# stardist/stardist

Hardware: AMD Instinct MI355X
Metric: predict_instances() Mpix/s (2D) + Mvox/s (3D) end-to-end at 1/2/4/8 GPU (higher is better)
Workload: dtype f32

## Files before the change

### stardist_amd/csrc/conv3x3_f16.hip

```cpp
#include <stdlib.h>

#include "common.h"
#include "conv3x3_device.h"
#include "stardist_hip.h"

#ifdef SD_CONV_PROFILE
__device__ unsigned long long g_conv_prof[20];
#define PROF_DECL unsigned long long pf_t = __builtin_amdgcn_s_memtime(), pf_acc[16] = {}; const unsigned long long pf_t0 = pf_t; unsigned long long pf_units = 0
#define PROF(k) do { const unsigned long long n_ = __builtin_amdgcn_s_memtime(); pf_acc[k] += n_ - pf_t; pf_t = n_; } while (0)
#define PROF_UNIT() (++pf_units)
#define PROF_END() do { if (threadIdx.x == 0) { atomicAdd(&g_conv_prof[0], __builtin_amdgcn_s_memtime() - pf_t0); \
  for (int k_ = 0; k_ < 16; ++k_) atomicAdd(&g_conv_prof[1 + k_], pf_acc[k_]); atomicAdd(&g_conv_prof[19], pf_units); } } while (0)
#else
#define PROF_DECL
#define PROF(k)
#define PROF_UNIT()
#define PROF_END()
#endif

#ifndef SD_CONV_EXP
#define SD_CONV_EXP 3
#endif

namespace {
// ... 90 lines not shown
  r.rsrc = __builtin_amdgcn_make_buffer_rsrc((void*)((k ? S1.p : S0.p) + (unsigned long long)(fl * 4)), 0, (int)HALO_RANGE, 0x00020000);
  r.ty0 = T.ty0; r.tx0 = T.tx0; r.H = zin ? d.H : 0; r.W = d.W;
  r.k = k; r.in = (int)(T.interior && zin);
  return r;
}

constexpr int WREG = (HWSUB_BYTES / 16 + THREADS - 1) / THREADS;
static_assert(WREG * THREADS == HWSUB_BYTES / 16, "a sub-unit's weights are a whole number of 16-byte elements per thread");
__device__ __forceinline__ void weights_fetch(const Params& P, int g, int u, int dy, v4f (&wreg)[WREG], int tid) {
  const char* blk = (const char*)P.wp + (((size_t)g * P.n_units + u) * 3 + dy) * HWSUB_BYTES;
  const __amdgpu_buffer_rsrc_t r = __builtin_amdgcn_make_buffer_rsrc((void*)uniform64((unsigned long long)blk), 0, HWSUB_BYTES, 0x00020000);
#pragma unroll
  for (int n = 0; n < WREG; ++n) wreg[n] = __builtin_bit_cast(v4f, __builtin_amdgcn_raw_buffer_load_b128(r, tid * 16, n * THREADS * 16, 0));
}
__device__ __forceinline__ void weights_store(char* __restrict__ wnext, const v4f (&wreg)[WREG], int tid) {
#pragma unroll
  for (int n = 0; n < WREG; ++n) ((v4f*)wnext)[tid + n * THREADS] = wreg[n];
}

__device__ __forceinline__ void split2_pair(float a, float b, unsigned& hi, unsigned& lo, float& amax) {
  const f32x2 x = {a, b};
  const f16x2 h = __builtin_convertvector(x, f16x2);
  hi = __builtin_bit_cast(unsigned, h);
  const f32x2 r = (x - __builtin_convertvector(h, f32x2)) * 2048.f;
  lo = __builtin_bit_cast(unsigned, __builtin_convertvector(r, f16x2));
  amax = __builtin_fmaxf(amax, __builtin_fmaxf(__builtin_fabsf(a), __builtin_fabsf(b)));
}
__device__ __forceinline__ void split_elem(const v4f x, u32x2 (&pl)[2], float& amax) {
  unsigned a[2], b[2];
  split2_pair(x.x, x.y, a[0], a[1], amax);
  split2_pair(x.z, x.w, b[0], b[1], amax);
#pragma unroll
  for (int p = 0; p < 2; ++p) {
    asm volatile("" : "+v"(a[p]), "+v"(b[p]));
    pl[p].x = a[p]; pl[p].y = b[p];
  }
}
__device__ __forceinline__ void store_planes(const StageH& st, char* __restrict__ tileH, const u32x2 (&pk)[PRE_F4][2], int tid) {
#pragma unroll
  for (int n = 0; n < PRE_F4; ++n)
    if (n < PRE_F4 - 1 || tid < TILE_F4 - (PRE_F4 - 1) * THREADS) {
#pragma unroll
      for (int p = 0; p < 2; ++p) *(u32x2*)(tileH + lds_off_of(st.tyx[n], tid) + p * 64) = pk[n][p];
    }
}

__device__ __forceinline__ void store_copy(const StageH& st, char* __restrict__ tileH, const v4f (&pre)[PRE_F4], int tid) {
#pragma unroll
  for (int n = 0; n < PRE_F4; ++n)
    if (n < PRE_F4 - 1 || tid < TILE_F4 - (PRE_F4 - 1) * THREADS) {
      const int pb = n < (TILE_F4 >> 8) ? 32 * n + ((tid >> 3) & 7) * 4 + ((tid >> 6) & 3) : (tid >> 3) + n * (THREADS / 8);
      *(v4f*)(tileH + pb * HPIX + (tid & 7) * 16) = pre[n];
    }
}

template <int NV, int NLD, class Extra>
__device__ __forceinline__ void compute_sub(const char* __restrict__ tileH, const char* __restrict__ w, int dy, f32x16 (&acc0)[2], f32x16 (&acc1)[2],
                                            int wave, int i, int h, Extra extra) {
  u32x4 A[2][2][2], B[2][2];
  const char* arow = tileH + (wave * 2 + dy) * HALO_W * HPIX;
#define SD_LOAD_GROUP_H(gi, buf)                                                                                        \
  do {                                                                                                                   \
    const int dx_ = (gi) >> 1, b_ = (gi) & 1;                                                                            \
    if (!(SD_CONV_EXP & 4) || (gi) < 2) {                                                                               \
    _Pragma("unroll") for (int p = 0; p < 2; ++p)                                                                        \
      _Pragma("unroll") for (int pl = 0; pl < 2; ++pl) A[buf][p][pl] = *(const u32x4*)(arow + htile_off(p, i + dx_, pl, b_, h)); \
    }                                                                                                                    \
    if (!(SD_CONV_EXP & 8) || (gi) < 2) {                                                                               \
    _Pragma("unroll") for (int pl = 0; pl < 2; ++pl) B[buf][pl] = *(const u32x4*)(w + hw_off(dx_, b_, pl, h, i));        \
    }                                                                                                                    \
  } while (0)
  SD_LOAD_GROUP_H(0, 0);
#pragma unroll
  for (int gi = 0; gi < 6; ++gi) {
    const int buf = gi & 1;
    if (gi + 1 < 6) SD_LOAD_GROUP_H(gi + 1, buf ^ 1);
    __builtin_amdgcn_sched_barrier(0);
    extra(gi);
    const f16x8 bh = __builtin_bit_cast(f16x8, B[buf][0]), bl = __builtin_bit_cast(f16x8, B[buf][1]);
    {
      const f16x8 a0h = __builtin_bit_cast(f16x8, A[buf][0][0]), a0l = __builtin_bit_cast(f16x8, A[buf][0][1]);
      const f16x8 a1h = __builtin_bit_cast(f16x8, A[buf][1][0]), a1l = __builtin_bit_cast(f16x8, A[buf][1][1]);
#if SD_CONV_EXP & 2
      acc1[0] = __builtin_amdgcn_mfma_f32_32x32x16_f16(a0h, bl, acc1[0], 0, 0, 0);
      acc1[1] = __builtin_amdgcn_mfma_f32_32x32x16_f16(a1h, bl, acc1[1], 0, 0, 0);
      acc0[0] = __builtin_amdgcn_mfma_f32_32x32x16_f16(a0h, bh, acc0[0], 0, 0, 0);
      acc1[0] = __builtin_amdgcn_mfma_f32_32x32x16_f16(a0l, bh, acc1[0], 0, 0, 0);
      acc1[1] = __builtin_amdgcn_mfma_f32_32x32x16_f16(a1l, bh, acc1[1], 0, 0, 0);
      acc0[1] = __builtin_amdgcn_mfma_f32_32x32x16_f16(a1h, bh, acc0[1], 0, 0, 0);
#else
      acc1[0] = __builtin_amdgcn_mfma_f32_32x32x16_f16(a0h, bl, acc1[0], 0, 0, 0);
      acc1[0] = __builtin_amdgcn_mfma_f32_32x32x16_f16(a0l, bh, acc1[0], 0, 0, 0);
      acc0[0] = __builtin_amdgcn_mfma_f32_32x32x16_f16(a0h, bh, acc0[0], 0, 0, 0);
      acc1[1] = __builtin_amdgcn_mfma_f32_32x32x16_f16(a1h, bl, acc1[1], 0, 0, 0);
      acc1[1] = __builtin_amdgcn_mfma_f32_32x32x16_f16(a1l, bh, acc1[1], 0, 0, 0);
      acc0[1] = __builtin_amdgcn_mfma_f32_32x32x16_f16(a1h, bh, acc0[1], 0, 0, 0);
#endif
    }
    if (NV > 0 || NLD > 0) {
#pragma unroll
      for (int k = 0; k < 6; ++k) {
        __builtin_amdgcn_sched_group_barrier(0x008, 1, 0);
        if (NV > 0) __builtin_amdgcn_sched_group_barrier(0x002, NV, 0);
        if (NLD > 0 && k % (6 / NLD) == 0) __builtin_amdgcn_sched_group_barrier(0x020, 1, 0);
      }
    }
    __builtin_amdgcn_sched_barrier(0);
  }
#undef SD_LOAD_GROUP_H
}

template <bool RES, bool DOT, bool NOST = false>
__device__ __forceinline__ void store_tile(const Params& P, const f32x16 (&acc0)[2], const f32x16 (&acc1)[2], float* __restrict__ scr, int g, int tz,
                                           int ty, int tx, int wave, int lane) {
  const int i = lane & 31, h = lane >> 5;
  const int px = lane >> 3, c4 = lane & 7;
  const unsigned pix_bytes = (unsigned)P.c_out * 4u, res_bytes = (unsigned)P.res_stride * 4u;
  const unsigned chan_off = (unsigned)(g * 32 + c4 * 4) * 4u;
#pragma unroll
  for (int p = 0; p < 2; ++p) {
    const int y = ty + wave * 2 + p;
    if (y >= P.H) continue;
    const size_t row = ((size_t)tz * P.H + y) * P.W;
    const __amdgpu_buffer_rsrc_t ro =
        __builtin_amdgcn_make_buffer_rsrc((void*)uniform64((unsigned long long)(P.out + row * P.c_out)), 0, (int)((unsigned)P.W * pix_bytes), 0x00020000);
    __amdgpu_buffer_rsrc_t rr = ro;
    if (RES && P.res)
      rr = __builtin_amdgcn_make_buffer_rsrc((void*)uniform64((unsigned long long)(P.res + row * P.res_stride)), 0, (int)((unsigned)P.W * res_bytes), 0x00020000);
    __amdgpu_buffer_rsrc_t rd = ro;
    if (DOT)
      rd = __builtin_amdgcn_make_buffer_rsrc((void*)uniform64((unsigned long long)(P.dotp + row * (size_t)(P.c_out >> 2))), 0, (int)((unsigned)P.W * (unsigned)P.c_out), 0x00020000);
#pragma unroll
    for (int q = 0; q < 2; ++q) {
#pragma unroll
      for (int r8 = 0; r8 < 8; ++r8) {
        const int r = q * 8 + r8;
        const int pl = (r8 & 3) + 8 * (r8 >> 2) + 4 * h;
        scr[pl * 32 + i] = acc0[p][r] + acc1[p][r] * 4.8828125e-4f;
      }
#pragma unroll
      for (int n = 0; n < 2; ++n) {
        v4f v = *(const v4f*)(scr + n * 256 + lane * 4);
        const unsigned x = (unsigned)(tx + q * 16 + n * 8 + px);
        if (RES && P.res) v += __builtin_bit_cast(v4f, __builtin_amdgcn_raw_buffer_load_b128(rr, (int)(x * res_bytes + chan_off), 0, 0));
        if (P.act == 1) { v.x = fmaxf(v.x, 0.f); v.y = fmaxf(v.y, 0.f); v.z = fmaxf(v.z, 0.f); v.w = fmaxf(v.w, 0.f); }
        const int so = (int)(x * pix_bytes + chan_off);
        if (!NOST) __builtin_amdgcn_raw_buffer_store_b128(__builtin_bit_cast(u32x4, v), ro, so, 0, 0);
        if (DOT) {
          const v4f hw = *(const v4f*)(scr + (4 - wave) * 512 + c4 * 4);
          float d = v.x * hw.x;
          d += v.y * hw.y; d += v.z * hw.z; d += v.w * hw.w;
          __builtin_amdgcn_raw_buffer_store_b32(__builtin_bit_cast(unsigned, d), rd, so >> 2, 0, 0);
        }
      }
    }
  }
}

__device__ __forceinline__ void store_tile_split(const Params& P, const f32x16 (&acc0)[2], const f32x16 (&acc1)[2], float* __restrict__ scr, int g, int tz,
                                                 int ty, int tx, int wave, int lane, float& amax) {
  const int i = lane & 31, h = lane >> 5;
  const int pr = lane >> 2, o = lane & 3;
  const unsigned pix_bytes = (unsigned)P.c_out * 4u;
  const unsigned chan_off = (unsigned)(g * 128 + o * 16);
  const int wofs = ((i >> 2) & 1) * 256 + (i >> 3) * 4 + (i & 3);
#pragma unroll
  for (int p = 0; p < 2; ++p) {
    const int y = ty + wave * 2 + p;
    if (y >= P.H) continue;
    const size_t row = ((size_t)tz * P.H + y) * P.W;
    const __amdgpu_buffer_rsrc_t ro =
        __builtin_amdgcn_make_buffer_rsrc((void*)uniform64((unsigned long long)(P.out + row * P.c_out)), 0, (int)((unsigned)P.W * pix_bytes), 0x00020000);
#pragma unroll
    for (int q = 0; q < 2; ++q) {
#pragma unroll
      for (int r8 = 0; r8 < 8; ++r8) {
        const int r = q * 8 + r8;
        const int pl = (r8 & 3) + 8 * (r8 >> 2) + 4 * h;
        scr[pl * 16 + wofs] = acc0[p][r] + acc1[p][r] * 4.8828125e-4f;
      }
      v4f va = *(const v4f*)(scr + lane * 4), vb = *(const v4f*)(scr + 256 + lane * 4);
      if (P.act == 1) {
        va.x = fmaxf(va.x, 0.f); va.y = fmaxf(va.y, 0.f); va.z = fmaxf(va.z, 0.f); va.w = fmaxf(va.w, 0.f);
        vb.x = fmaxf(vb.x, 0.f); vb.y = fmaxf(vb.y, 0.f); vb.z = fmaxf(vb.z, 0.f); vb.w = fmaxf(vb.w, 0.f);
      }
      unsigned hw[4], lw[4];
      split2_pair(va.x, va.y, hw[0], lw[0], amax);
      split2_pair(va.z, va.w, hw[1], lw[1], amax);
      split2_pair(vb.x, vb.y, hw[2], lw[2], amax);
      split2_pair(vb.z, vb.w, hw[3], lw[3], amax);
      const u32x4 hi = {hw[0], hw[1], hw[2], hw[3]}, lo = {lw[0], lw[1], lw[2], lw[3]};
      const int so = (int)((unsigned)(tx + q * 16 + pr) * pix_bytes + chan_off);
      __builtin_amdgcn_raw_buffer_store_b128(hi, ro, so, 0, 0);
      __builtin_amdgcn_raw_buffer_store_b128(lo, ro, so + 64, 0, 0);
    }
  }
}

template <bool RES, int WPE, bool DOT = false, bool INP = false, bool OUTP = false, bool NOST = false>
__global__ void __launch_bounds__(THREADS) __attribute__((amdgpu_waves_per_eu(WPE, WPE))) k_conv3_f16(const Params P) {
  static_assert(!(OUTP && (RES || DOT)), "a split16 output has neither residual nor fused head");
  static_assert(!NOST || DOT, "only the fused-head form can do without its tile store");
  extern __shared__ float4 smem4h[];
  char* W = (char*)smem4h;
  char* tileH = W + 2 * HWSUB_BYTES;
  const int tid = threadIdx.x, lane = tid & 63;
  const int wave = __builtin_amdgcn_readfirstlane(tid >> 6);
  float* scr = (float*)(tileH + HTILE_BYTES) + wave * 512;
  int g, q, Q;
  wg_slot(P, g, q, Q);
  if (q >= P.n_tiles) return;
  if (DOT && tid < 32) ((float*)(tileH + HTILE_BYTES) + 4 * 512)[tid] = P.dotw[g * 32 + tid];
  const float bias_r = P.bias ? P.bias[g * 32 + (lane & 31)] : 0.f;
  StageH st;
  stage_init_h(st, tid);
  const unsigned q4off = (unsigned)(tid & 7) * 16u;
  constexpr bool PREOFF = INP && (SD_CONV_EXP & 1);
  unsigned offk[PREOFF ? 2 : 1][PREOFF ? PRE_F4 : 1];
  if constexpr (PREOFF) {
#pragma unroll
    for (int k = 0; k < 2; ++k) {
      const Src S = P.kind[k];
      const unsigned rowb = (unsigned)((P.W >> S.shx) * S.stride * 4), pixb = (unsigned)(S.stride * 4);
#pragma unroll
      for (int n = 0; n < PRE_F4; ++n) {
        const int ty = (int)(st.tyx[n] & 255u), tx = (int)(st.tyx[n] >> 8);
        offk[k][n] = (unsigned)(((ty - S.shy) >> S.shy) + S.shy) * rowb + ((unsigned)(((tx - S.shx) >> S.shx) + S.shx) * pixb + q4off);
      }
    }
  }
  const SrcS S0 = src_scalars(P, 0), S1 = src_scalars(P, 1);
  DimS dim;
  dim.D = __builtin_amdgcn_readfirstlane(P.D); dim.H = __builtin_amdgcn_readfirstlane(P.H); dim.W = __builtin_amdgcn_readfirstlane(P.W);
  dim.kz = __builtin_amdgcn_readfirstlane(P.kz); dim.n0 = __builtin_amdgcn_readfirstlane(P.n_chunks0);
  TileAddr Tc, Tn;
  TileWalk walk;
  walk_init(P, q, Q, walk);
  tile_at(P, walk, Tc);
  Tn = Tc;
  float amax = 0.f, amax_out = 0.f;
  {
    v4f pre[PRE_F4], wreg[WREG];
    weights_fetch(P, g, 0, 0, wreg, tid);
    {
      const HaloRsrc hs = halo_rsrc(P, halo_base(P, Tc, 0), Tc);
#pragma unroll
      for (int n = 0; n < PRE_F4; ++n) pre[n] = halo_load_one(hs, halo_off_one(hs, st.tyx[n], q4off));
    }
    weights_store(W, wreg, tid);
    if (INP) store_copy(st, tileH, pre, tid);
    else {
      u32x2 pk[PRE_F4][2];
#pragma unroll
      for (int n = 0; n < PRE_F4; ++n) split_elem(pre[n], pk[n], amax);
      store_planes(st, tileH, pk, tid);
    }
  }
  __syncthreads();
  PROF_DECL;
  int wb = 0;
  for (int t = q; t < P.n_tiles; t += Q) {
    f32x16 acc0[2], acc1[2];
#pragma unroll
    for (int p = 0; p < 2; ++p)
#pragma unroll
      for (int r = 0; r < 16; ++r) { acc0[p][r] = bias_r; acc1[p][r] = 0.f; }
    for (int u = 0; u < P.n_units; ++u) {
      const bool last = u == P.n_units - 1;
      const int tn = last ? t + Q : t, un = last ? 0 : u + 1;
      const bool have = tn < P.n_tiles;
      v4f pre[PRE_F4];
      unsigned addr[PRE_F4];
      u32x2 pk[INP ? 1 : PRE_F4][2];
      HaloRsrc hs;
      UnitS us;
#pragma unroll
      for (int dy = 0; dy < 3; ++dy) {
        const bool lastdy = dy == 2, have_w = lastdy ? have : true;
        v4f wreg[WREG];
        weights_fetch(P, g, lastdy ? (have ? un : u) : u, lastdy ? (have ? 0 : dy) : dy + 1, wreg, tid);
        __builtin_amdgcn_sched_barrier(0);
        PROF(dy);
        if (!PREOFF && dy == 0 && last && have) { walk_step(P, walk); tile_at(P, walk, Tn); }
        __builtin_amdgcn_sched_barrier(0);
        if (dy == 0) PROF(14);
        const char* wcur = W + wb * HWSUB_BYTES;
        if (PREOFF && dy == 1 && !us.in) {
#pragma unroll
          for (int n = 0; n < PRE_F4; ++n) {
            const int ty = (int)(st.tyx[n] & 255u), tx = (int)(st.tyx[n] >> 8);
            const bool inside = (int)((unsigned)(us.ty0 + ty) < (unsigned)us.H) & (int)((unsigned)(us.tx0 + tx) < (unsigned)us.W);
            addr[n] = inside ? addr[n] : HALO_OUTSIDE;
          }
        }
        if (dy == 0 && PREOFF) {
          compute_sub<1, 0>(tileH, wcur, dy, acc0, acc1, wave, lane & 31, lane >> 5, [&](int gi) {
            if (gi == 0) {
              if (last && have) { walk_step(P, walk); tile_at_s(S0, S1, dim, walk, Tn); }
              us = unit_scalars(S0, S1, dim, tile_select(last && have, Tc, Tn), have ? un : u);
            } else {
              const bool k1 = us.k != 0;
#pragma unroll
              for (int n = (gi - 1) * 3; n < (gi - 1) * 3 + 3; ++n)
                if (n < PRE_F4) { unsigned a = k1 ? offk[1][PREOFF ? n : 0] : offk[0][PREOFF ? n : 0]; asm volatile("" : "+v"(a)); addr[n] = a; }
            }
          });
        } else if (dy == 0) {
          const TileAddr T = tile_select(last && have, Tc, Tn);
          const HaloBase hb = halo_base(P, T, have ? un : u);
          hs = halo_rsrc(P, hb, T);
          PROF(8);
          compute_sub<5, 0>(tileH, wcur, dy, acc0, acc1, wave, lane & 31, lane >> 5, [&](int gi) {
#pragma unroll
            for (int n = gi * 2; n < gi * 2 + 2; ++n)
              if (n < PRE_F4) addr[n] = halo_off_one(hs, st.tyx[n], q4off);
          });
        } else if (dy == 1) {
          compute_sub<0, 2>(tileH, wcur, dy, acc0, acc1, wave, lane & 31, lane >> 5, [&](int gi) {
#pragma unroll
            for (int n = gi * 2; n < gi * 2 + 2; ++n)
              if (n < PRE_F4) pre[n] = PREOFF ? __builtin_bit_cast(v4f, __builtin_amdgcn_raw_buffer_load_b128(us.rsrc, (int)addr[n], 0, 0)) : halo_load_one(hs, addr[n]);
          });
        } else if (INP) {
          compute_sub<0, 0>(tileH, wcur, dy, acc0, acc1, wave, lane & 31, lane >> 5, [&](int) {});
        } else {
          compute_sub<6, 0>(tileH, wcur, dy, acc0, acc1, wave, lane & 31, lane >> 5, [&](int gi) {
#pragma unroll
            for (int n = (gi - 2) * 3; n < (gi - 2) * 3 + 3; ++n)
              if (gi >= 2 && n < PRE_F4) split_elem(pre[n], pk[INP ? 0 : n], amax);
          });
        }
        PROF(dy == 0 ? 3 : 11 + dy);
        if (have_w) weights_store(W + (wb ^ 1) * HWSUB_BYTES, wreg, tid);
        if (lastdy) {
#pragma unroll
          for (int n = 0; n < WREG; ++n) asm volatile("" ::"v"(wreg[n]));
        }
        PROF(4 + dy);
        __syncthreads();
        PROF(7);
        wb ^= 1;
      }
      PROF(8);
      if (have) {
        if constexpr (INP) store_copy(st, tileH, pre, tid);
        else store_planes(st, tileH, pk, tid);
      }
      PROF(9);
      __syncthreads();
      PROF(10);
      PROF_UNIT();
    }
    if constexpr (OUTP) store_tile_split(P, acc0, acc1, scr, g, Tc.tz, Tc.ty0 + 1, Tc.tx0 + 1, wave, lane, amax_out);
    else store_tile<RES, DOT, NOST>(P, acc0, acc1, scr, g, Tc.tz, Tc.ty0 + 1, Tc.tx0 + 1, wave, lane);
    PROF(11);
    Tc = Tn;
  }
  if (!INP && P.flag && !(amax <= 65504.f)) atomicOr(P.flag, 1);
  if (OUTP && P.flag && !(amax_out <= 65504.f)) atomicOr(P.flag, 2);
  PROF_END();
}

struct RowsParams {
  const float* src; int c_in;
  int D, H, W, kz, n_units;
  const float* wp; const float* bias;
  int c_out, act, g0;
  const long long* rows; long long n_rows;
  float* out;
};
template <int NG, bool INP>
__global__ void __launch_bounds__(256) k_conv3_f16_rows(const RowsParams P) {
  extern __shared__ float4 rows_lds4[];
  char* wl = (char*)rows_lds4;
  const int tid = threadIdx.x, lane = tid & 63, i = lane & 31, h = lane >> 5;
  const long long wbase = ((long long)blockIdx.x * 4 + (tid >> 6)) * 32;
  const long long ri = wbase + i;
  const bool live = ri < P.n_rows;
  long long pix = live ? P.rows[ri] : 0;
  const int x = (int)(pix % P.W); pix /= P.W;
  const int y = (int)(pix % P.H);
  const int z = (int)(pix / P.H);
  f32x16 acc0[NG], acc1[NG];
#pragma unroll
  for (int g = 0; g < NG; ++g) {
    const float b = P.bias ? P.bias[(P.g0 + g) * 32 + i] : 0.f;
#pragma unroll
    for (int r = 0; r < 16; ++r) { acc0[g][r] = b; acc1[g][r] = 0.f; }
  }
  const size_t pix_floats = (size_t)P.c_in;
  float amax = 0.f;
  for (int u = 0; u < P.n_units; ++u) {
    const int c = P.kz == 3 ? u / 3 : u, dz = P.kz == 3 ? u - 3 * c - 1 : 0;
    const int zz = z + dz;
    const bool zin = live && zz >= 0 && zz < P.D;
    const int zc = min(max(zz, 0), P.D - 1);
#pragma unroll 1
    for (int dy = 0; dy < 3; ++dy) {
      const int yy = y + dy - 1;
      const bool yin = zin && yy >= 0 && yy < P.H;
      const int yc = min(max(yy, 0), P.H - 1);
      const float* prow = P.src + (((size_t)zc * P.H + yc) * P.W) * pix_floats + (size_t)c * 32;
      u32x4 ah[6], al[6];
      v4f f0[INP ? 1 : 6], f1[INP ? 1 : 6];
#pragma unroll
      for (int gi = 0; gi < 6; ++gi) {
        const int dx = gi >> 1, b = gi & 1;
        const int xc = min(max(x + dx - 1, 0), P.W - 1);
        const float* px = prow + (size_t)xc * pix_floats;
        if (INP) {
          ah[gi] = *(const u32x4*)(px + (b * 2 + h) * 4);
          al[gi] = *(const u32x4*)(px + 16 + (b * 2 + h) * 4);
        } else {
          f0[INP ? 0 : gi] = *(const v4f*)(px + b * 16 + h * 8); f1[INP ? 0 : gi] = *(const v4f*)(px + b * 16 + h * 8 + 4);
        }
      }
      __syncthreads();
#pragma unroll
      for (int g = 0; g < NG; ++g) {
        const v4f* wsrc = (const v4f*)((const char*)P.wp + ((((size_t)(P.g0 + g) * P.n_units + u) * 3 + dy) * HWSUB_BYTES));
#pragma unroll
        for (int n = 0; n < HWSUB_BYTES / 16 / 256; ++n) ((v4f*)(wl + g * HWSUB_BYTES))[tid + n * 256] = wsrc[tid + n * 256];
      }
      __syncthreads();
#pragma unroll
      for (int gi = 0; gi < 6; ++gi) {
        const int dx = gi >> 1, b = gi & 1;
        const int xx = x + dx - 1;
        const bool inside = yin && xx >= 0 && xx < P.W;
        u32x4 a_h, a_l;
        if (INP) { a_h = ah[gi]; a_l = al[gi]; }
        else {
          const v4f v0 = f0[INP ? 0 : gi], v1 = f1[INP ? 0 : gi];
          unsigned hw[4], lw[4];
          split2_pair(v0.x, v0.y, hw[0], lw[0], amax); split2_pair(v0.z, v0.w, hw[1], lw[1], amax);
          split2_pair(v1.x, v1.y, hw[2], lw[2], amax); split2_pair(v1.z, v1.w, hw[3], lw[3], amax);
          a_h = u32x4{hw[0], hw[1], hw[2], hw[3]}; a_l = u32x4{lw[0], lw[1], lw[2], lw[3]};
// ... 31 lines not shown

extern "C" int sd_conv3_f16x3_pack_weights_host(const float* w, int c_in, int c_out, int kz, float* packed) {
  const long long n = sd_conv3_f16x3_packed_floats(c_in, c_out, kz);
  if (!w || !packed || n < 0) {
    sd::set_error("sd_conv3_f16x3_pack_weights: kz 1|3, c_in a multiple of 32 up to 512, c_out a multiple of 32");
    return -1;
  }
  const float wmax = sdconv::pack_weights_f16(w, c_in, c_out, kz, (unsigned short*)packed);
  for (int k = 0; k < 4; ++k) packed[n - 4 + k] = 0.f;
  if (!(wmax <= 65504.f)) {
    sd::set_error("sd_conv3_f16x3_pack_weights: a weight of magnitude %g is outside the fp16 range (use the bf16x6 form for this layer)", (double)wmax);
    return -2;
  }
  return 0;
}

static int conv3_f16x3_launch(const float* d_src0, int c0, int stride0, int up0, const float* d_src1, int c1, int stride1,
                              int up1, int D, int H, int W, int kz, const float* d_wpacked, const float* d_bias,
                              const float* d_res, int res_stride, int c_out, int act, float* d_out, int* d_range_flag,
                              const float* d_dot_w, float* d_dot_partial, void* stream_, int in_split = 0, int out_split = 0) {
  hipStream_t s = (hipStream_t)stream_;
  const bool no_store = d_out == nullptr && d_dot_w != nullptr && d_dot_partial != nullptr && !d_res && !out_split;
  if ((in_split & ~1) || (out_split & ~1) || (out_split && (d_res || d_dot_w)) || (in_split && d_res) ||
      (in_split && (stride0 != c0 || (d_src1 && stride1 != c1)))) {
    sd::set_error("sd_conv3_f16x3: split16 tensors are dense (stride == channels); a split16 output takes neither residual nor fused head, a residual layer no split16 input");
    return -1;
  }
  if (D <= 0 || H <= 0 || W <= 0) return 0;
  const int c_in = c0 + (d_src1 ? c1 : 0);
  const long long n_packed = sd_conv3_f16x3_packed_floats(c_in, c_out, kz);
  if (!d_src0 || !d_wpacked || (!d_out && !no_store) || (act != 0 && act != 1) || n_packed < 0 || (kz == 1 && D != 1) ||
      (((uintptr_t)d_src0 | (uintptr_t)d_src1 | (uintptr_t)d_wpacked | (uintptr_t)d_out | (uintptr_t)d_bias) & 15) || ((uintptr_t)d_range_flag & 3)) {
    sd::set_error("sd_conv3_f16x3: unsupported channel counts (%d + %d -> %d), kz, act or misaligned pointers", c0, d_src1 ? c1 : 0, c_out);
    return -1;
  }
  const int ups[2] = {up0, d_src1 ? up1 : 0};
  for (int k = 0; k < 2; ++k)
    if (ups[k] < 0 || ups[k] > 7 || ((ups[k] & 1) && (W & 1)) || ((ups[k] & 2) && (H & 1)) || ((ups[k] & 4) && (D & 1))) {
      sd::set_error("sd_conv3_f16x3: up is a bit mask (1: x, 2: y, 4: z); an up-sampled axis needs an even output size");
      return -1;
    }
  if ((c0 % 32) || (d_src1 && (c1 % 32)) || stride0 < c0 || (stride0 & 3) || (d_src1 && (stride1 < c1 || (stride1 & 3)))) {
    sd::set_error("sd_conv3_f16x3: sources must hold multiples of 32 channels, strides multiples of 4 floats");
    return -1;
  }
  Params P;
  int nc = 0;
  P.kind[0] = make_src(d_src0, stride0, up0, H, W);
  P.kind[1] = d_src1 ? make_src(d_src1, stride1, up1, H, W) : P.kind[0];
  for (int k = 0; k < MAX_CHUNKS; ++k) { P.chunk_kind[k] = 0; P.chunk_choff[k] = 0; }
  for (int k = 0; k < c0 / 32; ++k) { P.chunk_kind[nc] = 0; P.chunk_choff[nc++] = k * 32; }
  if (d_src1) for (int k = 0; k < c1 / 32; ++k) { P.chunk_kind[nc] = 1; P.chunk_choff[nc++] = k * 32; }
  P.D = D; P.H = H; P.W = W; P.kz = kz; P.n_units = nc * kz; P.n_chunks0 = c0 / 32;
  P.zero = d_wpacked + (n_packed - 4);
  if (d_res && (res_stride < c_out || (res_stride & 3) || ((uintptr_t)d_res & 15))) {
    sd::set_error("sd_conv3_f16x3: the residual needs 16-byte alignment and a stride >= c_out");
    return -1;
  }
  P.res = d_res; P.res_stride = res_stride;
  P.wp = d_wpacked; P.bias = d_bias; P.out = d_out; P.c_out = c_out; P.act = act;
  P.flag = d_range_flag;
  if ((d_dot_w != nullptr) != (d_dot_partial != nullptr) || (d_dot_w && d_res) || ((uintptr_t)d_dot_w & 15) || ((uintptr_t)d_dot_partial & 3) ||
      (d_dot_w && (long long)W * c_out >= 0x7fffffffLL)) {
    sd::set_error("sd_conv3_f16x3: the fused head needs both its weights (16-byte aligned) and its partial-sum buffer, and no residual");
    return -1;
  }
  P.dotw = d_dot_w; P.dotp = d_dot_partial;
  P.tiles_x = (W + TW - 1) / TW;
  P.tiles_plane = P.tiles_x * ((H + TH - 1) / TH);
  const long long nt_ll = (long long)P.tiles_plane * D;
  if (nt_ll > 0x7fffffffLL) { sd::set_error("sd_conv3_f16x3: too many tiles"); return -1; }
  const long long row0 = (long long)(W >> (up0 & 1)) * stride0 * 4, row1 = d_src1 ? (long long)(W >> (up1 & 1)) * stride1 * 4 : 0;
  if ((HALO_H + 1) * (row0 > row1 ? row0 : row1) >= 0x7fffffffLL || (long long)W * c_out * 4 >= 0x7fffffffLL ||
      (d_res && (long long)W * res_stride * 4 >= 0x7fffffffLL)) {
    sd::set_error("sd_conv3_f16x3: an image row of %d pixels is too long for 32-bit offsets", W);
    return -1;
  }
  P.n_tiles = (int)nt_ll;
  P.groups = c_out / 32;
  static bool attr_set[16] = {};
  static int n_cu[16] = {};
  int dev = 0;
  SD_CHECK(hipGetDevice(&dev));
  const size_t lds = (size_t)2 * HWSUB_BYTES + HTILE_BYTES + 4 * 2048 + 128;
  typedef void (*kern_t)(const Params);
  static const kern_t kern[9][2] = {
      {k_conv3_f16<false, 2>, k_conv3_f16<false, 1>},
      {k_conv3_f16<true, 2>, k_conv3_f16<true, 1>},
      {k_conv3_f16<false, 2, true>, k_conv3_f16<false, 1, true>},
      {k_conv3_f16<false, 2, false, true, false>, k_conv3_f16<false, 1, false, true, false>},
      {k_conv3_f16<false, 2, false, false, true>, k_conv3_f16<false, 1, false, false, true>},
      {k_conv3_f16<false, 2, false, true, true>, k_conv3_f16<false, 1, false, true, true>},
      {k_conv3_f16<false, 2, true, true, false>, k_conv3_f16<false, 1, true, true, false>},
      {k_conv3_f16<false, 2, true, false, false, true>, k_conv3_f16<false, 1, true, false, false, true>},
      {k_conv3_f16<false, 2, true, true, false, true>, k_conv3_f16<false, 1, true, true, false, true>}};
  if (dev >= 16 || !attr_set[dev]) {
    for (int v = 0; v < 9; ++v)
      for (int w = 0; w < 2; ++w) SD_CHECK(hipFuncSetAttribute((const void*)kern[v][w], hipFuncAttributeMaxDynamicSharedMemorySize, (int)lds));
    if (dev < 16) attr_set[dev] = true;
  }
  int cus = dev < 16 ? n_cu[dev] : 0;
  if (cus <= 0) {
    SD_CHECK(hipDeviceGetAttribute(&cus, hipDeviceAttributeMultiprocessorCount, dev));
    if (cus <= 0) cus = 256;
    if (dev < 16) n_cu[dev] = cus;
  }
  const int per_cu = sd::option(sd::OPT_CONV_F16_WGS) == 1 ? 1 : 2;
  long long blocks = (long long)(per_cu * cus / P.groups) * P.groups;
  if (blocks < P.groups) blocks = P.groups;
  const long long want = (long long)P.n_tiles * P.groups;
  if (blocks > want) blocks = want;
  const int variant = d_dot_w ? ((in_split ? 6 : 2) + (no_store ? (in_split ? 2 : 5) : 0)) : d_res ? 1 : (in_split ? (out_split ? 5 : 3) : (out_split ? 4 : 0));
  hipLaunchKernelGGL(kern[variant][per_cu == 1 ? 1 : 0], dim3((unsigned)blocks), dim3(THREADS), lds, s, P);
  SD_LAUNCH_CHECK();
  return 0;
}

extern "C" int sd_conv3_f16x3_res_ndhwc_device(const float* d_src0, int c0, int stride0, int up0, const float* d_src1, int c1, int stride1,
                                               int up1, int D, int H, int W, int kz, const float* d_wpacked, const float* d_bias,
                                               const float* d_res, int res_stride, int c_out, int act, float* d_out, int* d_range_flag,
                                               void* stream_) {
  return conv3_f16x3_launch(d_src0, c0, stride0, up0, d_src1, c1, stride1, up1, D, H, W, kz, d_wpacked, d_bias, d_res, res_stride, c_out, act, d_out,
                            d_range_flag, nullptr, nullptr, stream_);
}

extern "C" int sd_conv3_f16x3_dot_ndhwc_device(const float* d_src0, int c0, int stride0, int up0, const float* d_src1, int c1, int stride1,
                                               int up1, int D, int H, int W, int kz, const float* d_wpacked, const float* d_bias, int c_out, int act,
                                               float* d_out, int* d_range_flag, const float* d_dot_w, float* d_dot_partial, void* stream_) {
  if (!d_dot_w || !d_dot_partial) { sd::set_error("sd_conv3_f16x3_dot: head weights and partial-sum buffer required"); return -1; }
  return conv3_f16x3_launch(d_src0, c0, stride0, up0, d_src1, c1, stride1, up1, D, H, W, kz, d_wpacked, d_bias, nullptr, 0, c_out, act, d_out,
                            d_range_flag, d_dot_w, d_dot_partial, stream_);
}

extern "C" int sd_conv3_f16x3_ndhwc_device(const float* d_src0, int c0, int stride0, int up0, const float* d_src1, int c1, int stride1, int up1,
                                           int D, int H, int W, int kz, const float* d_wpacked, const float* d_bias, int c_out, int act,
                                           float* d_out, int* d_range_flag, void* stream_) {
  return sd_conv3_f16x3_res_ndhwc_device(d_src0, c0, stride0, up0, d_src1, c1, stride1, up1, D, H, W, kz, d_wpacked, d_bias, nullptr, 0,
                                         c_out, act, d_out, d_range_flag, stream_);
}

extern "C" int sd_conv3_f16x3_fmt_ndhwc_device(const float* d_src0, int c0, int up0, const float* d_src1, int c1, int up1, int D, int H, int W, int kz,
                                               const float* d_wpacked, const float* d_bias, int c_out, int act, float* d_out, int in_split16,
                                               int out_split16, int* d_range_flag, const float* d_dot_w, float* d_dot_partial, void* stream_) {
  return conv3_f16x3_launch(d_src0, c0, c0, up0, d_src1, c1, c1, up1, D, H, W, kz, d_wpacked, d_bias, nullptr, 0, c_out, act, d_out, d_range_flag,
                            d_dot_w, d_dot_partial, stream_, in_split16 ? 1 : 0, out_split16 ? 1 : 0);
}

extern "C" int sd_conv3_f16x3_rows_device(const float* d_src, int c_in, int in_split16, int D, int H, int W, int kz, const float* d_wpacked,
                                          const float* d_bias, int c_out, int act, const long long* d_rows, long long n_rows, float* d_out,
                                          void* stream_) {
  hipStream_t s = (hipStream_t)stream_;
  if (n_rows <= 0) return 0;
  if (!d_src || !d_wpacked || !d_rows || !d_out || (act != 0 && act != 1) || sd_conv3_f16x3_packed_floats(c_in, c_out, kz) < 0 || (kz == 1 && D != 1) ||
      D <= 0 || H <= 0 || W <= 0 || (((uintptr_t)d_src | (uintptr_t)d_wpacked) & 15) || ((uintptr_t)d_rows & 7) || ((uintptr_t)d_out & 3)) {
    sd::set_error("sd_conv3_f16x3_rows: channel counts multiples of 32 (c_in <= 512), kz 1|3, act 0|1, aligned pointers");
    return -1;
  }
  RowsParams P;
  P.src = d_src; P.c_in = c_in; P.D = D; P.H = H; P.W = W; P.kz = kz; P.n_units = (c_in / 32) * kz;
  P.wp = d_wpacked; P.bias = d_bias; P.c_out = c_out; P.act = act; P.rows = d_rows; P.n_rows = n_rows; P.out = d_out;
  const long long waves = (n_rows + 31) / 32;
  const dim3 grid((unsigned)((waves + 3) / 4));
  const int groups = c_out / 32;
  for (int g0 = 0; g0 < groups;) {
    const int ng = groups - g0 >= 4 ? 4 : (groups - g0 >= 2 ? 2 : 1);
    P.g0 = g0;
    const size_t lds = (size_t)ng * HWSUB_BYTES;
// ... 15 lines not shown
```

### stardist_amd/csrc/conv3x3_layout.h

```cpp
#pragma once
#include <stddef.h>

#if defined(__HIPCC__)
#define SDC_HD __host__ __device__ inline
#else
#define SDC_HD inline
#endif

namespace sdconv {

constexpr int TH = 8, TW = 32;
constexpr int HALO_H = TH + 2, HALO_W = TW + 2;
constexpr int CHUNK = 32;
constexpr int PIX_STRIDE = 36;
constexpr int TILE_FLOATS = HALO_H * HALO_W * PIX_STRIDE;
constexpr int TILE_F4 = HALO_H * HALO_W * (CHUNK / 4);
constexpr int THREADS = 256;
constexpr int PRE_F4 = (TILE_F4 + THREADS - 1) / THREADS;
constexpr int MAX_CHUNKS = 16;

SDC_HD int nt_for(int c_out) { (void)c_out; return 1; }
SDC_HD int wunit_floats(int nt) { return 9 * 4 * 2 * 32 * nt * 4; }
SDC_HD size_t packed_floats(int c_in, int c_out, int kz) { return (size_t)c_out * c_in * 9 * kz; }
SDC_HD int chan_of(int j, int h, int e) { return h * 16 + j * 4 + e; }
SDC_HD size_t wpack_index(int g, int u, int tap, int j, int h, int n, int e, int n_units, int nt) {
  return ((((((size_t)g * n_units + u) * 9 + tap) * 4 + j) * 2 + h) * (32 * nt) + n) * 4 + e;
}
SDC_HD int wl_off(int tap, int j, int h, int ct, int i, int nt) { return (((tap * 4 + j) * 2 + h) * (32 * nt) + ct * 32 + i) * 4; }
SDC_HD int tile_off(int ty, int tx, int ch) { return (ty * HALO_W + tx) * PIX_STRIDE + ch; }
SDC_HD int a_off(int row, int dy, int dx, int j, int i, int h) { return tile_off(row + dy, i + dx, h * 16 + j * 4); }
SDC_HD int acc_col(int r, int h) { return (r & 3) + 8 * (r >> 2) + 4 * h; }
SDC_HD void stage_elem(int e, int& ty, int& tx, int& q4) {
  const int pix = e >> 3;
  q4 = e & 7;
  ty = pix / HALO_W;
  tx = pix - ty * HALO_W;
}

SDC_HD void stage_elem_b(int e, int& ty, int& tx, int& q4) {
  q4 = e & 7;
  const int n = e >> 8;
  const int pix = n < (TILE_F4 >> 8) ? 32 * n + ((e >> 3) & 7) * 4 + ((e >> 6) & 3) : e >> 3;
  ty = pix / HALO_W;
  tx = pix - ty * HALO_W;
}

SDC_HD int src_rel(int t, int sh) { return sh ? ((t - 1) >> 1) + 1 : t; }
SDC_HD int src_base(int t0, int sh) { return sh ? ((t0 + 1) >> 1) - 1 : t0; }

inline void pack_weights(const float* w, int c_in, int c_out, int kz, float* out) {
  const int nt = nt_for(c_out), n_chunks = c_in / CHUNK, groups = c_out / (32 * nt), n_units = n_chunks * kz;
  for (int g = 0; g < groups; ++g)
    for (int c = 0; c < n_chunks; ++c)
      for (int z = 0; z < kz; ++z)
        for (int tap = 0; tap < 9; ++tap)
          for (int j = 0; j < 4; ++j)
            for (int h = 0; h < 2; ++h)
              for (int n = 0; n < 32 * nt; ++n)
                for (int e = 0; e < 4; ++e) {
                  const int co = g * 32 * nt + n, ci = c * CHUNK + chan_of(j, h, e);
                  out[wpack_index(g, c * kz + z, tap, j, h, n, e, n_units, nt)] = w[(((size_t)co * c_in + ci) * kz + z) * 9 + tap];
                }
}

constexpr int BPIX = 208;
constexpr int BTILE_BYTES = HALO_H * HALO_W * BPIX;
constexpr int BWSUB_BYTES = 3 * 2 * 3 * 2 * 32 * 16;
SDC_HD int btile_off(int ty, int tx, int p, int b, int h) { return (ty * HALO_W + tx) * BPIX + p * 64 + b * 32 + h * 16; }
SDC_HD int btile_store_off(int ty, int tx, int p, int q4) { return (ty * HALO_W + tx) * BPIX + p * 64 + q4 * 8; }
SDC_HD int bw_off(int dx, int b, int p, int h, int i) { return ((((dx * 2 + b) * 3 + p) * 2 + h) * 32 + i) * 16; }
SDC_HD size_t bpacked_bytes(int c_in, int c_out, int kz) { return (size_t)(c_out / 32) * (c_in / CHUNK) * kz * 3 * BWSUB_BYTES; }

SDC_HD unsigned f2u(float f) { unsigned u; __builtin_memcpy(&u, &f, 4); return u; }
SDC_HD float u2f(unsigned u) { float f; __builtin_memcpy(&f, &u, 4); return f; }
SDC_HD unsigned bf16_bits(float f) { unsigned u = f2u(f); u += 0x7FFFu + ((u >> 16) & 1u); return u & 0xFFFF0000u; }
SDC_HD void split3(float x, unsigned& hi, unsigned& mid, unsigned& lo) {
  hi = bf16_bits(x);
  const float r = x - u2f(hi);
  mid = bf16_bits(r);
  lo = bf16_bits(r - u2f(mid));
}

inline void pack_weights_bf16(const float* w, int c_in, int c_out, int kz, unsigned short* out) {
  const int n_chunks = c_in / CHUNK, groups = c_out / 32, n_units = n_chunks * kz;
  for (int g = 0; g < groups; ++g)
    for (int c = 0; c < n_chunks; ++c)
      for (int z = 0; z < kz; ++z)
        for (int dy = 0; dy < 3; ++dy)
          for (int dx = 0; dx < 3; ++dx)
            for (int b = 0; b < 2; ++b)
              for (int h = 0; h < 2; ++h)
                for (int i = 0; i < 32; ++i)
                  for (int j = 0; j < 8; ++j) {
                    const int co = g * 32 + i, ci = c * CHUNK + b * 16 + h * 8 + j;
                    unsigned pl[3];
                    split3(w[(((size_t)co * c_in + ci) * kz + z) * 9 + dy * 3 + dx], pl[0], pl[1], pl[2]);
                    const size_t sub = (((size_t)g * n_units + c * kz + z) * 3 + dy) * BWSUB_BYTES;
                    for (int p = 0; p < 3; ++p) out[(sub + bw_off(dx, b, p, h, i)) / 2 + j] = (unsigned short)(pl[p] >> 16);
                  }
}

constexpr int HPIX = 144;
constexpr int HTILE_BYTES = HALO_H * HALO_W * HPIX;
constexpr int HWSUB_BYTES = 3 * 2 * 2 * 2 * 32 * 16;
SDC_HD int htile_off(int ty, int tx, int p, int b, int h) { return (ty * HALO_W + tx) * HPIX + p * 64 + b * 32 + h * 16; }
SDC_HD int htile_store_off(int ty, int tx, int p, int q4) { return (ty * HALO_W + tx) * HPIX + p * 64 + q4 * 8; }
SDC_HD int hw_off(int dx, int b, int p, int h, int i) { return ((((dx * 2 + b) * 2 + p) * 2 + h) * 32 + i) * 16; }
SDC_HD size_t hpacked_bytes(int c_in, int c_out, int kz) { return (size_t)(c_out / 32) * (c_in / CHUNK) * kz * 3 * HWSUB_BYTES; }

SDC_HD unsigned short f16_bits(float f) {
  const unsigned u = f2u(f), sign = (u >> 16) & 0x8000u, a = u & 0x7FFFFFFFu;
  if (a >= 0x7F800000u) return (unsigned short)(sign | 0x7C00u | ((a > 0x7F800000u) ? 0x200u : 0u));
  if (a >= 0x477FF000u) return (unsigned short)(sign | 0x7C00u);
  if (a < 0x33000001u) return (unsigned short)sign;
  int e = (int)(a >> 23) - 127;
  unsigned m = (a & 0x7FFFFFu) | 0x800000u;
  int shift = e >= -14 ? 13 : 13 + (-14 - e);
  const unsigned keep = m >> shift, rem = m & ((1u << shift) - 1u), half = 1u << (shift - 1);
  unsigned r = keep + ((rem > half || (rem == half && (keep & 1u))) ? 1u : 0u);
  const unsigned bits = e >= -14 ? ((unsigned)(e + 14) << 10) + r : r;
  return (unsigned short)(sign | bits);
}
SDC_HD float f16_value(unsigned short h) {
  const unsigned sign = (unsigned)(h & 0x8000u) << 16, e = (h >> 10) & 31u, m = h & 0x3FFu;
  if (e == 31u) return u2f(sign | 0x7F800000u | (m << 13));
  if (e == 0u) {
    float v = (float)m * 5.9604644775390625e-08f;
    return (sign ? -v : v);
  }
  return u2f(sign | ((e + 112u) << 23) | (m << 13));
}
SDC_HD void split2_f16(float x, unsigned short& hi, unsigned short& lo) {
  hi = f16_bits(x);
  lo = f16_bits((x - f16_value(hi)) * 2048.f);
}

inline float pack_weights_f16(const float* w, int c_in, int c_out, int kz, unsigned short* out) {
  const int n_chunks = c_in / CHUNK, groups = c_out / 32, n_units = n_chunks * kz;
  float wmax = 0.f;
  for (int g = 0; g < groups; ++g)
    for (int c = 0; c < n_chunks; ++c)
      for (int z = 0; z < kz; ++z)
        for (int dy = 0; dy < 3; ++dy)
          for (int dx = 0; dx < 3; ++dx)
            for (int b = 0; b < 2; ++b)
              for (int h = 0; h < 2; ++h)
                for (int i = 0; i < 32; ++i)
                  for (int j = 0; j < 8; ++j) {
                    const int co = g * 32 + i, ci = c * CHUNK + b * 16 + h * 8 + j;
                    const float x = w[(((size_t)co * c_in + ci) * kz + z) * 9 + dy * 3 + dx];
                    const float ax = x < 0 ? -x : x;
                    if (!(ax <= wmax)) wmax = ax;
                    unsigned short pl[2];
                    split2_f16(x, pl[0], pl[1]);
                    const size_t sub = (((size_t)g * n_units + c * kz + z) * 3 + dy) * HWSUB_BYTES;
                    for (int p = 0; p < 2; ++p) out[(sub + hw_off(dx, b, p, h, i)) / 2 + j] = pl[p];
                  }
  return wmax;
}

}
```

Measured before the change: 313.0.

## Swap MFMA operands so accumulators hold pixel-major layout, drop LDS transpose in epilogue

The MFMA A/B operands are swapped, so each lane's accumulator now holds channels of one pixel rather than pixels of one channel. The store epilogues can then write output directly from registers, or via permlane32_swap for the split path, instead of transposing through an LDS scratch area. Bias and dot weights move into a small LDS tail, and the per-wave scratch allocation is removed, which shrinks LDS use and may allow higher occupancy. The cost is per-lane strided global stores and bias loaded from LDS at each tile start.

```diff
diff --git a/stardist_amd/csrc/conv3x3_f16.hip b/stardist_amd/csrc/conv3x3_f16.hip
--- a/stardist_amd/csrc/conv3x3_f16.hip
+++ b/stardist_amd/csrc/conv3x3_f16.hip
@@ -196,19 +196,19 @@
       const f16x8 a0h = __builtin_bit_cast(f16x8, A[buf][0][0]), a0l = __builtin_bit_cast(f16x8, A[buf][0][1]);
       const f16x8 a1h = __builtin_bit_cast(f16x8, A[buf][1][0]), a1l = __builtin_bit_cast(f16x8, A[buf][1][1]);
 #if SD_CONV_EXP & 2
-      acc1[0] = __builtin_amdgcn_mfma_f32_32x32x16_f16(a0h, bl, acc1[0], 0, 0, 0);
-      acc1[1] = __builtin_amdgcn_mfma_f32_32x32x16_f16(a1h, bl, acc1[1], 0, 0, 0);
-      acc0[0] = __builtin_amdgcn_mfma_f32_32x32x16_f16(a0h, bh, acc0[0], 0, 0, 0);
-      acc1[0] = __builtin_amdgcn_mfma_f32_32x32x16_f16(a0l, bh, acc1[0], 0, 0, 0);
-      acc1[1] = __builtin_amdgcn_mfma_f32_32x32x16_f16(a1l, bh, acc1[1], 0, 0, 0);
-      acc0[1] = __builtin_amdgcn_mfma_f32_32x32x16_f16(a1h, bh, acc0[1], 0, 0, 0);
+      acc1[0] = __builtin_amdgcn_mfma_f32_32x32x16_f16(bl, a0h, acc1[0], 0, 0, 0);
+      acc1[1] = __builtin_amdgcn_mfma_f32_32x32x16_f16(bl, a1h, acc1[1], 0, 0, 0);
+      acc0[0] = __builtin_amdgcn_mfma_f32_32x32x16_f16(bh, a0h, acc0[0], 0, 0, 0);
+      acc1[0] = __builtin_amdgcn_mfma_f32_32x32x16_f16(bh, a0l, acc1[0], 0, 0, 0);
+      acc1[1] = __builtin_amdgcn_mfma_f32_32x32x16_f16(bh, a1l, acc1[1], 0, 0, 0);
+      acc0[1] = __builtin_amdgcn_mfma_f32_32x32x16_f16(bh, a1h, acc0[1], 0, 0, 0);
 #else
-      acc1[0] = __builtin_amdgcn_mfma_f32_32x32x16_f16(a0h, bl, acc1[0], 0, 0, 0);
-      acc1[0] = __builtin_amdgcn_mfma_f32_32x32x16_f16(a0l, bh, acc1[0], 0, 0, 0);
-      acc0[0] = __builtin_amdgcn_mfma_f32_32x32x16_f16(a0h, bh, acc0[0], 0, 0, 0);
-      acc1[1] = __builtin_amdgcn_mfma_f32_32x32x16_f16(a1h, bl, acc1[1], 0, 0, 0);
-      acc1[1] = __builtin_amdgcn_mfma_f32_32x32x16_f16(a1l, bh, acc1[1], 0, 0, 0);
-      acc0[1] = __builtin_amdgcn_mfma_f32_32x32x16_f16(a1h, bh, acc0[1], 0, 0, 0);
+      acc1[0] = __builtin_amdgcn_mfma_f32_32x32x16_f16(bl, a0h, acc1[0], 0, 0, 0);
+      acc1[0] = __builtin_amdgcn_mfma_f32_32x32x16_f16(bh, a0l, acc1[0], 0, 0, 0);
+      acc0[0] = __builtin_amdgcn_mfma_f32_32x32x16_f16(bh, a0h, acc0[0], 0, 0, 0);
+      acc1[1] = __builtin_amdgcn_mfma_f32_32x32x16_f16(bl, a1h, acc1[1], 0, 0, 0);
+      acc1[1] = __builtin_amdgcn_mfma_f32_32x32x16_f16(bh, a1l, acc1[1], 0, 0, 0);
+      acc0[1] = __builtin_amdgcn_mfma_f32_32x32x16_f16(bh, a1h, acc0[1], 0, 0, 0);
 #endif
     }
     if (NV > 0 || NLD > 0) {
@@ -225,12 +225,18 @@
 }
 
 template <bool RES, bool DOT, bool NOST = false>
-__device__ __forceinline__ void store_tile(const Params& P, const f32x16 (&acc0)[2], const f32x16 (&acc1)[2], float* __restrict__ scr, int g, int tz,
+__device__ __forceinline__ void store_tile(const Params& P, const f32x16 (&acc0)[2], const f32x16 (&acc1)[2], const float* __restrict__ tail, int g, int tz,
                                            int ty, int tx, int wave, int lane) {
   const int i = lane & 31, h = lane >> 5;
-  const int px = lane >> 3, c4 = lane & 7;
   const unsigned pix_bytes = (unsigned)P.c_out * 4u, res_bytes = (unsigned)P.res_stride * 4u;
-  const unsigned chan_off = (unsigned)(g * 32 + c4 * 4) * 4u;
+  const unsigned chan_off = (unsigned)(g * 32 + h * 4) * 4u;
+  const unsigned x = (unsigned)(tx + i);
+  const int so = (int)(x * pix_bytes + chan_off);
+  v4f hw[DOT ? 4 : 1];
+  if (DOT) {
+#pragma unroll
+    for (int k = 0; k < 4; ++k) hw[DOT ? k : 0] = *(const v4f*)(tail + 32 + k * 8 + h * 4);
+  }
 #pragma unroll
   for (int p = 0; p < 2; ++p) {
     const int y = ty + wave * 2 + p;
@@ -244,40 +250,38 @@
     __amdgpu_buffer_rsrc_t rd = ro;
     if (DOT)
       rd = __builtin_amdgcn_make_buffer_rsrc((void*)uniform64((unsigned long long)(P.dotp + row * (size_t)(P.c_out >> 2))), 0, (int)((unsigned)P.W * (unsigned)P.c_out), 0x00020000);
-#pragma unroll
-    for (int q = 0; q < 2; ++q) {
-#pragma unroll
-      for (int r8 = 0; r8 < 8; ++r8) {
-        const int r = q * 8 + r8;
-        const int pl = (r8 & 3) + 8 * (r8 >> 2) + 4 * h;
-        scr[pl * 32 + i] = acc0[p][r] + acc1[p][r] * 4.8828125e-4f;
-      }
-#pragma unroll
-      for (int n = 0; n < 2; ++n) {
-        v4f v = *(const v4f*)(scr + n * 256 + lane * 4);
-        const unsigned x = (unsigned)(tx + q * 16 + n * 8 + px);
-        if (RES && P.res) v += __builtin_bit_cast(v4f, __builtin_amdgcn_raw_buffer_load_b128(rr, (int)(x * res_bytes + chan_off), 0, 0));
-        if (P.act == 1) { v.x = fmaxf(v.x, 0.f); v.y = fmaxf(v.y, 0.f); v.z = fmaxf(v.z, 0.f); v.w = fmaxf(v.w, 0.f); }
-        const int so = (int)(x * pix_bytes + chan_off);
-        if (!NOST) __builtin_amdgcn_raw_buffer_store_b128(__builtin_bit_cast(u32x4, v), ro, so, 0, 0);
-        if (DOT) {
-          const v4f hw = *(const v4f*)(scr + (4 - wave) * 512 + c4 * 4);
-          float d = v.x * hw.x;
-          d += v.y * hw.y; d += v.z * hw.z; d += v.w * hw.w;
-          __builtin_amdgcn_raw_buffer_store_b32(__builtin_bit_cast(unsigned, d), rd, so >> 2, 0, 0);
-        }
-      }
-    }
-  }
-}
-
-__device__ __forceinline__ void store_tile_split(const Params& P, const f32x16 (&acc0)[2], const f32x16 (&acc1)[2], float* __restrict__ scr, int g, int tz,
+    v4f res[RES ? 4 : 1];
+    if (RES && P.res) {
+#pragma unroll
+      for (int k = 0; k < 4; ++k)
+        res[RES ? k : 0] = __builtin_bit_cast(v4f, __builtin_amdgcn_raw_buffer_load_b128(rr, (int)(x * res_bytes + chan_off) + k * 32, 0, 0));
+    }
+#pragma unroll
+    for (int k = 0; k < 4; ++k) {
+      v4f v;
+      v.x = acc0[p][k * 4 + 0] + acc1[p][k * 4 + 0] * 4.8828125e-4f;
+      v.y = acc0[p][k * 4 + 1] + acc1[p][k * 4 + 1] * 4.8828125e-4f;
+      v.z = acc0[p][k * 4 + 2] + acc1[p][k * 4 + 2] * 4.8828125e-4f;
+      v.w = acc0[p][k * 4 + 3] + acc1[p][k * 4 + 3] * 4.8828125e-4f;
+      if (RES && P.res) v += res[RES ? k : 0];
+      if (P.act == 1) { v.x = fmaxf(v.x, 0.f); v.y = fmaxf(v.y, 0.f); v.z = fmaxf(v.z, 0.f); v.w = fmaxf(v.w, 0.f); }
+      if (!NOST) __builtin_amdgcn_raw_buffer_store_b128(__builtin_bit_cast(u32x4, v), ro, so + k * 32, 0, 0);
+      if (DOT) {
+        const v4f w4 = hw[DOT ? k : 0];
+        float d = v.x * w4.x;
+        d += v.y * w4.y; d += v.z * w4.z; d += v.w * w4.w;
+        __builtin_amdgcn_raw_buffer_store_b32(__builtin_bit_cast(unsigned, d), rd, (so >> 2) + k * 8, 0, 0);
+      }
+    }
+  }
+}
+
+__device__ __forceinline__ void store_tile_split(const Params& P, const f32x16 (&acc0)[2], const f32x16 (&acc1)[2], int g, int tz,
                                                  int ty, int tx, int wave, int lane, float& amax) {
   const int i = lane & 31, h = lane >> 5;
-  const int pr = lane >> 2, o = lane & 3;
   const unsigned pix_bytes = (unsigned)P.c_out * 4u;
-  const unsigned chan_off = (unsigned)(g * 128 + o * 16);
-  const int wofs = ((i >> 2) & 1) * 256 + (i >> 3) * 4 + (i & 3);
+  const unsigned chan_off = (unsigned)(g * 128 + h * 16);
+  const int so = (int)((unsigned)(tx + i) * pix_bytes + chan_off);
 #pragma unroll
   for (int p = 0; p < 2; ++p) {
     const int y = ty + wave * 2 + p;
@@ -286,27 +290,25 @@
     const __amdgpu_buffer_rsrc_t ro =
         __builtin_amdgcn_make_buffer_rsrc((void*)uniform64((unsigned long long)(P.out + row * P.c_out)), 0, (int)((unsigned)P.W * pix_bytes), 0x00020000);
 #pragma unroll
-    for (int q = 0; q < 2; ++q) {
-#pragma unroll
-      for (int r8 = 0; r8 < 8; ++r8) {
-        const int r = q * 8 + r8;
-        const int pl = (r8 & 3) + 8 * (r8 >> 2) + 4 * h;
-        scr[pl * 16 + wofs] = acc0[p][r] + acc1[p][r] * 4.8828125e-4f;
-      }
-      v4f va = *(const v4f*)(scr + lane * 4), vb = *(const v4f*)(scr + 256 + lane * 4);
+    for (int kk = 0; kk < 2; ++kk) {
+      float v[8];
+#pragma unroll
+      for (int j = 0; j < 4; ++j) {
+        const float a = acc0[p][kk * 8 + j] + acc1[p][kk * 8 + j] * 4.8828125e-4f;
+        const float b = acc0[p][kk * 8 + 4 + j] + acc1[p][kk * 8 + 4 + j] * 4.8828125e-4f;
+        const u32x2 s = __builtin_amdgcn_permlane32_swap(__builtin_bit_cast(unsigned, a), __builtin_bit_cast(unsigned, b), false, false);
+        v[j] = __builtin_bit_cast(float, s.x); v[4 + j] = __builtin_bit_cast(float, s.y);
+      }
       if (P.act == 1) {
-        va.x = fmaxf(va.x, 0.f); va.y = fmaxf(va.y, 0.f); va.z = fmaxf(va.z, 0.f); va.w = fmaxf(va.w, 0.f);
-        vb.x = fmaxf(vb.x, 0.f); vb.y = fmaxf(vb.y, 0.f); vb.z = fmaxf(vb.z, 0.f); vb.w = fmaxf(vb.w, 0.f);
+#pragma unroll
+        for (int j = 0; j < 8; ++j) v[j] = fmaxf(v[j], 0.f);
       }
       unsigned hw[4], lw[4];
-      split2_pair(va.x, va.y, hw[0], lw[0], amax);
-      split2_pair(va.z, va.w, hw[1], lw[1], amax);
-      split2_pair(vb.x, vb.y, hw[2], lw[2], amax);
-      split2_pair(vb.z, vb.w, hw[3], lw[3], amax);
+#pragma unroll
+      for (int j = 0; j < 4; ++j) split2_pair(v[2 * j], v[2 * j + 1], hw[j], lw[j], amax);
       const u32x4 hi = {hw[0], hw[1], hw[2], hw[3]}, lo = {lw[0], lw[1], lw[2], lw[3]};
-      const int so = (int)((unsigned)(tx + q * 16 + pr) * pix_bytes + chan_off);
-      __builtin_amdgcn_raw_buffer_store_b128(hi, ro, so, 0, 0);
-      __builtin_amdgcn_raw_buffer_store_b128(lo, ro, so + 64, 0, 0);
+      __builtin_amdgcn_raw_buffer_store_b128(hi, ro, so + kk * 32, 0, 0);
+      __builtin_amdgcn_raw_buffer_store_b128(lo, ro, so + kk * 32 + 64, 0, 0);
     }
   }
 }
@@ -320,12 +322,12 @@
   char* tileH = W + 2 * HWSUB_BYTES;
   const int tid = threadIdx.x, lane = tid & 63;
   const int wave = __builtin_amdgcn_readfirstlane(tid >> 6);
-  float* scr = (float*)(tileH + HTILE_BYTES) + wave * 512;
+  float* tail = (float*)(tileH + HTILE_BYTES);
   int g, q, Q;
   wg_slot(P, g, q, Q);
   if (q >= P.n_tiles) return;
-  if (DOT && tid < 32) ((float*)(tileH + HTILE_BYTES) + 4 * 512)[tid] = P.dotw[g * 32 + tid];
-  const float bias_r = P.bias ? P.bias[g * 32 + (lane & 31)] : 0.f;
+  if (tid < 32) tail[tid] = P.bias ? P.bias[g * 32 + tid] : 0.f;
+  if (DOT && tid < 32) tail[32 + tid] = P.dotw[g * 32 + tid];
   StageH st;
   stage_init_h(st, tid);
   const unsigned q4off = (unsigned)(tid & 7) * 16u;
@@ -376,9 +378,18 @@
   for (int t = q; t < P.n_tiles; t += Q) {
     f32x16 acc0[2], acc1[2];
 #pragma unroll
-    for (int p = 0; p < 2; ++p)
-#pragma unroll
-      for (int r = 0; r < 16; ++r) { acc0[p][r] = bias_r; acc1[p][r] = 0.f; }
+    for (int p = 0; p < 2; ++p) {
+      int boff = (lane >> 5) * 4;
+      asm volatile("" : "+v"(boff));
+#pragma unroll
+      for (int k = 0; k < 4; ++k) {
+        const v4f b4 = *(const v4f*)(tail + k * 8 + boff);
+        acc0[p][k * 4 + 0] = b4.x; acc0[p][k * 4 + 1] = b4.y; acc0[p][k * 4 + 2] = b4.z; acc0[p][k * 4 + 3] = b4.w;
+      }
+#pragma unroll
+      for (int r = 0; r < 16; ++r) acc1[p][r] = 0.f;
+    }
+    __builtin_assume(P.n_units > 0);
     for (int u = 0; u < P.n_units; ++u) {
       const bool last = u == P.n_units - 1;
       const int tn = last ? t + Q : t, un = last ? 0 : u + 1;
@@ -465,8 +476,8 @@
       PROF(10);
       PROF_UNIT();
     }
-    if constexpr (OUTP) store_tile_split(P, acc0, acc1, scr, g, Tc.tz, Tc.ty0 + 1, Tc.tx0 + 1, wave, lane, amax_out);
-    else store_tile<RES, DOT, NOST>(P, acc0, acc1, scr, g, Tc.tz, Tc.ty0 + 1, Tc.tx0 + 1, wave, lane);
+    if constexpr (OUTP) store_tile_split(P, acc0, acc1, g, Tc.tz, Tc.ty0 + 1, Tc.tx0 + 1, wave, lane, amax_out);
+    else store_tile<RES, DOT, NOST>(P, acc0, acc1, tail, g, Tc.tz, Tc.ty0 + 1, Tc.tx0 + 1, wave, lane);
     PROF(11);
     Tc = Tn;
   }
@@ -664,7 +675,7 @@
   static int n_cu[16] = {};
   int dev = 0;
   SD_CHECK(hipGetDevice(&dev));
-  const size_t lds = (size_t)2 * HWSUB_BYTES + HTILE_BYTES + 4 * 2048 + 128;
+  const size_t lds = (size_t)2 * HWSUB_BYTES + HTILE_BYTES + 256;
   typedef void (*kern_t)(const Params);
   static const kern_t kern[9][2] = {
       {k_conv3_f16<false, 2>, k_conv3_f16<false, 1>},
diff --git a/stardist_amd/csrc/conv3x3_layout.h b/stardist_amd/csrc/conv3x3_layout.h
--- a/stardist_amd/csrc/conv3x3_layout.h
+++ b/stardist_amd/csrc/conv3x3_layout.h
@@ -106,6 +106,7 @@
 SDC_HD int htile_off(int ty, int tx, int p, int b, int h) { return (ty * HALO_W + tx) * HPIX + p * 64 + b * 32 + h * 16; }
 SDC_HD int htile_store_off(int ty, int tx, int p, int q4) { return (ty * HALO_W + tx) * HPIX + p * 64 + q4 * 8; }
 SDC_HD int hw_off(int dx, int b, int p, int h, int i) { return ((((dx * 2 + b) * 2 + p) * 2 + h) * 32 + i) * 16; }
+SDC_HD int acc_chan(int r, int h) { return 8 * (r >> 2) + 4 * h + (r & 3); }
 SDC_HD size_t hpacked_bytes(int c_in, int c_out, int kz) { return (size_t)(c_out / 32) * (c_in / CHUNK) * kz * 3 * HWSUB_BYTES; }
 
 SDC_HD unsigned short f16_bits(float f) {
```

Result: slower. 224.3 (-28.3%).
